# anilkeshwani/speech-integration

Hardware: AMD Instinct MI355X
Metric: train_tokens_per_sec (higher is better)
Workload: dtype bf16; 1 GPU; Llama-3.2-1B +5000 DSUs (V=133258), SFT step fwd+bwd+AdamW, seq_len=2048, batch=8/GPU, grad_accum=1, 16 layers, random-init weights, MLS-shaped synthetic DSU sequences; global_batch=8, seq_len=2048, parallelism=dp1

## Files before the change

speech-integration_amd/csrc/embed_ce.hip:

```cpp
#include "common_hip.h"

template <typename T>
__global__ __launch_bounds__(256) void embed_fwd_kernel(const int64_t* __restrict__ tokens, const T* __restrict__ table,
                                                        T* __restrict__ out, int64_t n_tok, int dim, int64_t vocab) {
    constexpr int N = Vec16<T>::N;
    const int nvec = dim / N;
    for (int64_t t = blockIdx.x; t < n_tok; t += gridDim.x) {
        const int64_t tok = tokens[t];
        const bool ok = tok >= 0 && tok < vocab;
        for (int v = threadIdx.x; v < nvec; v += 256) {
            Vec16<T> a;
            if (ok) a = load16(table + tok * dim + v * N);
            else
#pragma unroll
                for (int i = 0; i < N; ++i) a.set(i, 0.f);
            store16(out + t * dim + v * N, a);
        }
    }
}

extern "C" int ssi_embed_fwd(const int64_t* tokens, const void* table, void* out, int64_t n_tok, int64_t dim,
                             int64_t vocab, int dtype, void* stream) {
    if (n_tok == 0) return SSI_OK;
    SSI_CHECK_ARG(tokens && table && out && n_tok > 0 && dim > 0 && dim % 8 == 0 && vocab > 0);
    const unsigned grid = (unsigned)(n_tok < 65536 ? n_tok : 65536);
    SSI_DISPATCH_DTYPE(dtype, hipLaunchKernelGGL(embed_fwd_kernel<T>, dim3(grid), dim3(256), 0, (hipStream_t)stream, tokens,
                                                 (const T*)table, (T*)out, n_tok, (int)dim, vocab));
    SSI_LAUNCH_CHECK();
    return SSI_OK;
}

__global__ __launch_bounds__(256) void embed_index_kernel(const int64_t* __restrict__ tokens, int64_t n_tok, int64_t vocab,
                                                          int* __restrict__ first, int* __restrict__ count) {
    const int64_t t = (int64_t)blockIdx.x * 256 + threadIdx.x;
    if (t >= n_tok) return;
    const int64_t tok = tokens[t];
    if (tok < 0 || tok >= vocab) return;
    atomicMin(&first[tok], (int)t);
    atomicAdd(&count[tok], 1);
}

template <typename T, int MAXV>
__global__ __launch_bounds__(256) void embed_bwd_kernel(const int64_t* __restrict__ tokens, const T* __restrict__ dout,
                                                        T* __restrict__ dtable, int64_t n_tok, int dim, int64_t vocab,
                                                        const int* __restrict__ first, const int* __restrict__ count) {
    constexpr int N = Vec16<T>::N;
    const int lane = threadIdx.x & 63;
    const int64_t t0 = (int64_t)blockIdx.x * 4 + (threadIdx.x >> 6);
    if (t0 >= n_tok) return;
    const int64_t tok = tokens[t0];
    if (tok < 0 || tok >= vocab) return;
    if (first[tok] != (int)t0) return;
    const int need = count[tok];
    const int nvec = dim / N;
    float acc[MAXV][N];
#pragma unroll
    for (int k = 0; k < MAXV; ++k)
#pragma unroll
        for (int i = 0; i < N; ++i) acc[k][i] = 0.f;
    constexpr int SCAN = 8, ROWS = 8;
    __shared__ int hits_lds[4][64 * SCAN];
    int* hits = hits_lds[threadIdx.x >> 6];
    int found = 0;
    for (int64_t base0 = (t0 / 64) * 64; base0 < n_tok && found < need; base0 += 64 * SCAN) {
        int64_t tk[SCAN];
#pragma unroll
        for (int u = 0; u < SCAN; ++u) {
            const int64_t idx = base0 + 64 * u + lane;
            tk[u] = tokens[idx < n_tok ? idx : n_tok - 1];
        }
        int n = 0;
#pragma unroll
        for (int u = 0; u < SCAN; ++u) {
            const int64_t idx = base0 + 64 * u + lane;
            const bool hit = idx < n_tok && idx >= t0 && tk[u] == tok;
            const unsigned long long mask = __ballot(hit);
            if (hit) hits[n + __popcll(mask & ((1ull << lane) - 1ull))] = (int)(idx - base0);
            n += __popcll(mask);
        }
        __builtin_amdgcn_s_waitcnt(0xc07f);
        if (n == 1) {
            const T* src = dout + (base0 + hits[0]) * dim;
#pragma unroll
            for (int k = 0; k < MAXV; ++k) {
                const int v = lane + k * 64;
                const Vec16<T> r = load16(src + (v < nvec ? v : nvec - 1) * N);
#pragma unroll
                for (int i = 0; i < N; ++i) acc[k][i] += v < nvec ? r.get(i) : 0.f;
            }
        } else
        for (int h0 = 0; h0 < n; h0 += ROWS) {
            int pos[ROWS];
#pragma unroll
            for (int u = 0; u < ROWS; ++u) pos[u] = hits[h0 + u < n ? h0 + u : n - 1];
            Vec16<T> a[ROWS][MAXV];
#pragma unroll
            for (int u = 0; u < ROWS; ++u) {
                const T* src = dout + (base0 + pos[u]) * dim;
#pragma unroll
                for (int k = 0; k < MAXV; ++k) {
                    const int v = lane + k * 64;
                    a[u][k] = load16(src + (v < nvec ? v : nvec - 1) * N);
                }
            }
            __builtin_amdgcn_sched_barrier(0);
#pragma unroll
            for (int u = 0; u < ROWS; ++u) {
                const bool row_ok = h0 + u < n;
#pragma unroll
                for (int k = 0; k < MAXV; ++k) {
                    const bool ok = row_ok && lane + k * 64 < nvec;
#pragma unroll
                    for (int i = 0; i < N; ++i) acc[k][i] += ok ? a[u][k].get(i) : 0.f;
                }
            }
        }
        found += n;
    }
    T* dst = dtable + tok * dim;
#pragma unroll
    for (int k = 0; k < MAXV; ++k) {
        const int v = lane + k * 64;
        if (v < nvec) {
            Vec16<T> a = load16(dst + v * N);
#pragma unroll
            for (int i = 0; i < N; ++i) a.set(i, a.get(i) + acc[k][i]);
            store16(dst + v * N, a);
        }
    }
}

static inline int64_t embed_ws_vocab_slots(int64_t vocab) { return ssi_align_up(vocab, 64); }
extern "C" int64_t ssi_embed_bwd_workspace_bytes(int64_t vocab) { return 2 * embed_ws_vocab_slots(vocab) * (int64_t)sizeof(int); }

template <typename T>
static int launch_embed_bwd(const int64_t* tokens, const T* dout, T* dtable, int64_t n_tok, int dim, int64_t vocab,
                            const int* first, const int* count, hipStream_t st) {
    const int64_t vec_per_lane = ssi_cdiv(dim / Vec16<T>::N, 64);
    const dim3 grid((unsigned)ssi_cdiv(n_tok, 4));
    if (vec_per_lane <= 1) hipLaunchKernelGGL((embed_bwd_kernel<T, 1>), grid, dim3(256), 0, st, tokens, dout, dtable, n_tok, dim, vocab, first, count);
    else if (vec_per_lane <= 2) hipLaunchKernelGGL((embed_bwd_kernel<T, 2>), grid, dim3(256), 0, st, tokens, dout, dtable, n_tok, dim, vocab, first, count);
    else if (vec_per_lane <= 4) hipLaunchKernelGGL((embed_bwd_kernel<T, 4>), grid, dim3(256), 0, st, tokens, dout, dtable, n_tok, dim, vocab, first, count);
    else if (vec_per_lane <= 8) hipLaunchKernelGGL((embed_bwd_kernel<T, 8>), grid, dim3(256), 0, st, tokens, dout, dtable, n_tok, dim, vocab, first, count);
    else { ssi_set_error("embed_bwd: dim %d too large", dim); return SSI_ERR_UNSUPPORTED; }
    return SSI_OK;
}

extern "C" int ssi_embed_bwd(const int64_t* tokens, const void* dout, void* dtable, int64_t n_tok, int64_t dim,
                             int64_t vocab, int dtype, void* workspace, int64_t workspace_bytes, void* stream) {
    if (n_tok == 0) return SSI_OK;
    SSI_CHECK_ARG(tokens && dout && dtable && n_tok > 0 && n_tok < (1LL << 31) && dim > 0 && dim % 8 == 0 && vocab > 0);
    if (!workspace || workspace_bytes < ssi_embed_bwd_workspace_bytes(vocab)) { ssi_set_error("embed_bwd: workspace too small"); return SSI_ERR_WORKSPACE; }
    auto st = (hipStream_t)stream;
    int* first = (int*)workspace;
    int* count = first + embed_ws_vocab_slots(vocab);
    hipError_t e = hipMemsetAsync(first, 0x7f, embed_ws_vocab_slots(vocab) * sizeof(int), st);
    if (e == hipSuccess) e = hipMemsetAsync(count, 0, embed_ws_vocab_slots(vocab) * sizeof(int), st);
    if (e != hipSuccess) { ssi_set_error("embed_bwd: memset failed: %s", hipGetErrorString(e)); return SSI_ERR_HIP + (int)e; }
    hipLaunchKernelGGL(embed_index_kernel, dim3((unsigned)ssi_cdiv(n_tok, 256)), dim3(256), 0, st, tokens, n_tok, vocab, first, count);
    SSI_LAUNCH_CHECK();
    int rc = SSI_OK;
    SSI_DISPATCH_DTYPE(dtype, rc = launch_embed_bwd<T>(tokens, (const T*)dout, (T*)dtable, n_tok, (int)dim, vocab, first, count, st));
    if (rc) return rc;
    SSI_LAUNCH_CHECK();
    return SSI_OK;
}

enum CeMode { CE_PLAIN, CE_Z, CE_SMOOTH, CE_METRICS, CE_KL };

struct CeKl {
    const void* teacher = nullptr; int64_t ld_teacher = 0; const float* teacher_lse = nullptr; const float* row_kl_weight = nullptr;
    float beta = 0.f; float* row_kl = nullptr;
};

__device__ __forceinline__ bool ce_label_valid(int64_t label, int64_t vocab, int64_t ignore_index) {
    return label != ignore_index && label >= 0 && label < vocab;
}

template <typename T> __device__ __forceinline__ void ce_zero_row(T* lr, int64_t nvec) {
    constexpr int N = Vec16<T>::N;
    Vec16<T> z;
#pragma unroll
    for (int i = 0; i < N; ++i) z.set(i, 0.f);
    for (int64_t v = threadIdx.x; v < nvec; v += 512) store16(lr + v * N, z);
}

template <typename T> __device__ __forceinline__ float ce_row_lse(const T* lr, int64_t nvec, int64_t vocab, float* red) {
    constexpr int N = Vec16<T>::N;
    float m = -INFINITY, s = 0.f;
    for (int64_t v = threadIdx.x; v < nvec; v += 512) {
        Vec16<T> a = load16(lr + v * N);
        float lm = -INFINITY;
#pragma unroll
        for (int i = 0; i < N; ++i) if (v * N + i < vocab) lm = fmaxf(lm, a.get(i));
        if (lm > m) { s *= expf(m - lm); m = lm; }
#pragma unroll
        for (int i = 0; i < N; ++i) if (v * N + i < vocab) s += expf(a.get(i) - m);
    }
    const float gm = block_max(m, red);
    s = (m == -INFINITY) ? 0.f : s * expf(m - gm);
    const float gs = block_sum(s, red);
    return gm + logf(gs);
}

template <typename T> __device__ __forceinline__ float ce_row_sum(const T* lr, int64_t nvec, int64_t vocab, float* red) {
    constexpr int N = Vec16<T>::N;
    float s = 0.f;
    for (int64_t v = threadIdx.x; v < nvec; v += 512) {
        Vec16<T> a = load16(lr + v * N);
#pragma unroll
        for (int i = 0; i < N; ++i) if (v * N + i < vocab) s += a.get(i);
    }
    return block_sum(s, red);
}

template <typename T> __device__ __forceinline__ int ce_rank_row(const T* lr, int64_t nvec, int64_t vocab, int64_t label, float xl, int* redi) {
    constexpr int N = Vec16<T>::N;
    int cnt = 0;
    for (int64_t v = threadIdx.x; v < nvec; v += 512) {
        Vec16<T> a = load16(lr + v * N);
#pragma unroll
        for (int i = 0; i < N; ++i) {
            const int64_t c = v * N + i;
            const float x = a.get(i);
            cnt += (int)(c < vocab) & ((int)(x > xl) | ((int)(x == xl) & (int)(c < label)));
        }
    }
    return block_sum_i32(cnt, redi);
}

template <CeMode MODE, typename T>
__device__ __forceinline__ void ce_grad_row(T* lr, int64_t nvec, int64_t vocab, int64_t label, float lse, float w, float f, float ome, float wu) {
    constexpr int N = Vec16<T>::N;
    for (int64_t v = threadIdx.x; v < nvec; v += 512) {
        Vec16<T> a = load16(lr + v * N), o;
#pragma unroll
        for (int i = 0; i < N; ++i) {
            const int64_t c = v * N + i;
            float g = 0.f;
            if (c < vocab) {
                if constexpr (MODE == CE_PLAIN) g = w * (expf(a.get(i) - lse) - (c == label ? 1.f : 0.f));
                else g = w * (f * expf(a.get(i) - lse) - (c == label ? ome : 0.f));
                if constexpr (MODE == CE_SMOOTH) {
                    asm volatile("" : "+v"(g));
                    g -= wu;
                }
            }
            o.set(i, g);
        }
        store16(lr + v * N, o);
    }
}

template <typename T>
__device__ __forceinline__ void ce_kl_row(T* lr, const T* tr, int64_t nvec, int64_t nvec_t, int64_t vocab, int64_t label, float lse, float tlse,
                                          float w, float bk, int write_grad, double (&acc)[3]) {
    constexpr int N = Vec16<T>::N;
    acc[0] = acc[1] = acc[2] = 0.0;
    for (int64_t v = threadIdx.x; v < nvec; v += 512) {
        Vec16<T> a = load16(lr + v * N), o;
        Vec16<T> b = a;
        if (v < nvec_t) b = load16(tr + v * N);
#pragma unroll
        for (int i = 0; i < N; ++i) {
            const int64_t c = v * N + i;
            float g = 0.f;
            if (c < vocab) {
                const float x = a.get(i), t = b.get(i);
                const float p = expf(x - lse), q = expf(t - tlse);
                const double Q = exp((double)t - (double)tlse);
                acc[0] += Q * ((double)t - (double)x);
                acc[1] += Q;
                acc[2] += exp((double)x - (double)lse);
                g = w * (p - (c == label ? 1.f : 0.f)) + bk * (p - q);
            }
            o.set(i, g);
        }
        if (write_grad) store16(lr + v * N, o);
    }
}

template <typename T, CeMode MODE>
__device__ __forceinline__ void ce_generic_body(T* __restrict__ logits, int64_t ld, const int64_t* __restrict__ labels, int64_t vocab,
                                                int64_t ignore_index, float two_z, float ome, float e_over_v, float* __restrict__ row_loss,
                                                float* __restrict__ row_lse, float* __restrict__ row_z, float* __restrict__ row_u,
                                                float* __restrict__ row_nll, int32_t* __restrict__ row_rank, int write_grad,
                                                const float* __restrict__ row_weight, float* red, int* redi, const CeKl& kl = CeKl{}) {
    const int64_t row = blockIdx.x;
    T* lr = logits + row * ld;
    const int64_t label = labels[row];
    const int64_t nvec = ld / Vec16<T>::N;
    const bool valid = ce_label_valid(label, vocab, ignore_index);
    float lse = 0.f, sx = 0.f, w = 1.f, xl = 0.f;
    int cnt = -1;
    if (valid) {
        lse = ce_row_lse(lr, nvec, vocab, red);
        if constexpr (MODE == CE_SMOOTH) sx = ce_row_sum(lr, nvec, vocab, red);
        w = row_weight ? row_weight[row] : 1.f;
        if (MODE == CE_METRICS || threadIdx.x == 0) xl = to_f32<T>(lr[label]);
        if constexpr (MODE == CE_METRICS) cnt = ce_rank_row(lr, nvec, vocab, label, xl, redi);
    }
    if (threadIdx.x == 0) {
        row_loss[row] = w * (lse - xl);
        if (row_lse) row_lse[row] = lse;
        if constexpr (MODE == CE_Z) row_z[row] = w * (lse * lse);
        if constexpr (MODE == CE_SMOOTH) {
            if (row_z) row_z[row] = w * (lse * lse);
            row_u[row] = w * (lse - sx / (float)vocab);
        }
        if constexpr (MODE == CE_METRICS) { row_nll[row] = lse - xl; row_rank[row] = cnt; }
    }
    if constexpr (MODE == CE_KL) {
        if (!valid) {
            if (threadIdx.x == 0) kl.row_kl[row] = 0.f;
            if (write_grad) ce_zero_row(lr, nvec);
            return;
        }
        const float kw = kl.row_kl_weight ? kl.row_kl_weight[row] : w;
        __syncthreads();
        const float tlse = kl.teacher_lse[row];
        double acc[3];
        ce_kl_row<T>(lr, (const T*)kl.teacher + row * kl.ld_teacher, nvec, kl.ld_teacher / Vec16<T>::N, vocab, label, lse, tlse, w, kl.beta * kw,
                     write_grad, acc);
        __shared__ double redd[3][8];
#pragma unroll
        for (int q = 0; q < 3; ++q) acc[q] = wave_sum_f64(acc[q]);
        if ((threadIdx.x & 63) == 0) {
#pragma unroll
            for (int q = 0; q < 3; ++q) redd[q][threadIdx.x >> 6] = acc[q];
        }
        __syncthreads();
        if (threadIdx.x == 0) {
            double sum[3] = {0.0, 0.0, 0.0};
            for (int q = 0; q < 3; ++q)
                for (int i = 0; i < 8; ++i) sum[q] += redd[q][i];
            kl.row_kl[row] = kw * (float)(sum[0] / sum[1] - ((double)tlse - (double)lse) - log(sum[1]) + log(sum[2]));
        }
    } else if constexpr (MODE != CE_METRICS) {
        if (!write_grad) return;
        if (!valid) { ce_zero_row(lr, nvec); return; }
        const float f = fmaf(two_z, lse, 1.f);
        __syncthreads();
        ce_grad_row<MODE>(lr, nvec, vocab, label, lse, w, f, ome, w * e_over_v);
    }
}

template <typename T>
__global__ __launch_bounds__(512) void ce_fwd_kernel(T* __restrict__ logits, int64_t ld, const int64_t* __restrict__ labels,
                                                     int64_t vocab, int64_t ignore_index, float* __restrict__ row_loss,
                                                     float* __restrict__ row_lse, int write_grad, const float* __restrict__ row_weight) {
    __shared__ float red[16];
    ce_generic_body<T, CE_PLAIN>(logits, ld, labels, vocab, ignore_index, 0.f, 1.f, 0.f, row_loss, row_lse, nullptr, nullptr, nullptr, nullptr,
                                 write_grad, row_weight, red, nullptr);
}

template <typename T>
__global__ __launch_bounds__(512) void ce_fwd_z_kernel(T* __restrict__ logits, int64_t ld, const int64_t* __restrict__ labels,
                                                       int64_t vocab, int64_t ignore_index, float two_z, float* __restrict__ row_loss,
                                                       float* __restrict__ row_lse, float* __restrict__ row_z, int write_grad,
                                                       const float* __restrict__ row_weight) {
    __shared__ float red[16];
    ce_generic_body<T, CE_Z>(logits, ld, labels, vocab, ignore_index, two_z, 1.f, 0.f, row_loss, row_lse, row_z, nullptr, nullptr, nullptr,
                             write_grad, row_weight, red, nullptr);
}

template <typename T>
__global__ __launch_bounds__(512) void ce_fwd_smooth_kernel(T* __restrict__ logits, int64_t ld, const int64_t* __restrict__ labels,
                                                            int64_t vocab, int64_t ignore_index, float two_z, float ome, float e_over_v,
                                                            float* __restrict__ row_loss, float* __restrict__ row_lse,
                                                            float* __restrict__ row_z, float* __restrict__ row_u, int write_grad,
                                                            const float* __restrict__ row_weight) {
    __shared__ float red[16];
    ce_generic_body<T, CE_SMOOTH>(logits, ld, labels, vocab, ignore_index, two_z, ome, e_over_v, row_loss, row_lse, row_z, row_u, nullptr, nullptr,
                                  write_grad, row_weight, red, nullptr);
}

template <typename T>
__global__ __launch_bounds__(512) void ce_fwd_metrics_kernel(const T* __restrict__ logits, int64_t ld, const int64_t* __restrict__ labels,
                                                             int64_t vocab, int64_t ignore_index, float* __restrict__ row_loss,
                                                             float* __restrict__ row_lse, float* __restrict__ row_nll,
                                                             int32_t* __restrict__ row_rank, const float* __restrict__ row_weight) {
    __shared__ float red[16];
    __shared__ int redi[16];
    ce_generic_body<T, CE_METRICS>(const_cast<T*>(logits), ld, labels, vocab, ignore_index, 0.f, 1.f, 0.f, row_loss, row_lse, nullptr, nullptr,
                                   row_nll, row_rank, 0, row_weight, red, redi);
}

template <typename T>
__global__ __launch_bounds__(512) void ce_kl_generic_kernel(T* __restrict__ logits, int64_t ld, const int64_t* __restrict__ labels,
                                                            int64_t vocab, int64_t ignore_index, CeKl kl, float* __restrict__ row_loss,
                                                            float* __restrict__ row_lse, int write_grad,
                                                            const float* __restrict__ row_weight) {
    __shared__ float red[16];
    ce_generic_body<T, CE_KL>(logits, ld, labels, vocab, ignore_index, 0.f, 1.f, 0.f, row_loss, row_lse, nullptr, nullptr, nullptr, nullptr,
                              write_grad, row_weight, red, nullptr, kl);
}


template <int NCH, CeMode MODE, bool write_grad>
__device__ __forceinline__ void ce_row_bf16_body(bf16_t* __restrict__ logits, int64_t ld, const int64_t* __restrict__ labels, int64_t rows,
                                                 int64_t vocab, int64_t ignore_index, float two_z, float ome, float e_over_v,
                                                 float* __restrict__ row_loss, float* __restrict__ row_lse, float* __restrict__ row_z,
                                                 float* __restrict__ row_u, float* __restrict__ row_nll, int32_t* __restrict__ row_rank,
                                                 const float* __restrict__ row_weight, float* red, int* redi, const CeKl& kl = CeKl{}) {
    static_assert(MODE != CE_METRICS || !write_grad, "the metrics form writes no gradient");
    constexpr bool KL = MODE == CE_KL;
    constexpr int TD = NCH < 3 ? NCH : 3;
    constexpr bool WITH_F = MODE == CE_Z || MODE == CE_SMOOTH;
    constexpr bool SMOOTH = MODE == CE_SMOOTH;
    constexpr float LOG2E = 1.44269504088896340736f;
    constexpr int CHUNK = 8192;
    const int tid = threadIdx.x;
    const int voff = tid * 16;
    const int col0 = tid * 8;
    const int row_bytes = (int)(ld * 2);
    const int vocab_i = (int)vocab;
    u32x4 x[NCH];
    auto rsrc_of = [&](int64_t row) { return __builtin_amdgcn_make_buffer_rsrc(logits + row * ld, 0, row_bytes, 0x00020000u); };
    [[maybe_unused]] u32x4 tq[TD];
    auto lo = [](unsigned u) { return __builtin_bit_cast(float, u << 16); };
    auto hi = [](unsigned u) { return __builtin_bit_cast(float, u & 0xffff0000u); };
    auto opaque = [&]() {
#pragma unroll
        for (int c = 0; c < NCH; ++c)
#pragma unroll
            for (int d = 0; d < 4; ++d) asm volatile("" : "+v"(x[c][d]));
    };
    int64_t row = blockIdx.x;
    if (row >= rows) return;
    {
        const __amdgpu_buffer_rsrc_t r0 = rsrc_of(row);
#pragma unroll
        for (int c = 0; c < NCH; ++c) x[c] = __builtin_amdgcn_raw_buffer_load_b128(r0, voff, c * CHUNK * 2, 0);
    }
    for (; row < rows; row += gridDim.x) {
        const int64_t next = row + gridDim.x;
        const int64_t label = labels[row];
        const bool valid = ce_label_valid(label, vocab, ignore_index);
        const float w = row_weight ? row_weight[row] : 1.f;
        float log2w = row_weight ? __log2f(w) : 0.f;
        const __amdgpu_buffer_rsrc_t rs = rsrc_of(row);
        [[maybe_unused]] float kw = 0.f, bk = 0.f, dl = 0.f, nq = -INFINITY, klacc = 0.f;
        [[maybe_unused]] __amdgpu_buffer_rsrc_t rt = rs;
        if constexpr (KL) {
            kw = kl.row_kl_weight ? kl.row_kl_weight[row] : w;
            rt = __builtin_amdgcn_make_buffer_rsrc(const_cast<bf16_t*>((const bf16_t*)kl.teacher) + row * ld, 0, row_bytes, 0x00020000u);
        }
#pragma unroll
        for (int c = (NCH >= 2 ? NCH - 2 : 0); c < NCH; ++c) {
            const int left = vocab_i - c * CHUNK - col0;
#pragma unroll
            for (int d = 0; d < 4; ++d) {
                if (2 * d >= left) x[c][d] = (x[c][d] & 0xffff0000u) | 0x0000ff80u;
                if (2 * d + 1 >= left) x[c][d] = (x[c][d] & 0x0000ffffu) | 0xff800000u;
            }
        }
        float nl = -INFINITY;
        float wl = w;
        float wus = 0.f;
        unsigned flip = 0u;
        if (valid) {
            float xl = 0.f;
            if (MODE == CE_METRICS || tid == 0) xl = (float)logits[row * ld + label];
            float m = -INFINITY;
#pragma unroll
            for (int c = 0; c < NCH; ++c)
#pragma unroll
                for (int d = 0; d < 4; ++d) m = fmaxf(m, fmaxf(lo(x[c][d]), hi(x[c][d])));
            if constexpr (MODE != CE_METRICS) asm volatile("s_waitcnt vmcnt(0)" ::: "memory");
            const float gm = block_max(m, red);
            if constexpr (KL) {
#pragma unroll
                for (int i = 0; i < TD; ++i) tq[i] = __builtin_amdgcn_raw_buffer_load_b128(rt, voff, i * CHUNK * 2, 2 );
            }
            opaque();
            const float nm = -gm * LOG2E;
            float s = 0.f;
#pragma unroll
            for (int c = 0; c < NCH; ++c)
#pragma unroll
                for (int d = 0; d < 4; ++d)
                    s += __builtin_amdgcn_exp2f(fmaf(lo(x[c][d]), LOG2E, nm)) + __builtin_amdgcn_exp2f(fmaf(hi(x[c][d]), LOG2E, nm));
            const float gs = block_sum(s, red);
            const float lse = gm + logf(gs);
            float gsx = 0.f;
            if constexpr (SMOOTH) {
                opaque();
                float sx = 0.f;
#pragma unroll
                for (int c = 0; c < NCH; ++c) {
                    const int left = vocab_i - c * CHUNK - col0;
#pragma unroll
                    for (int d = 0; d < 4; ++d) {
                        if (c < NCH - 2) sx += lo(x[c][d]) + hi(x[c][d]);
                        else sx += (2 * d < left ? lo(x[c][d]) : 0.f) + (2 * d + 1 < left ? hi(x[c][d]) : 0.f);
                    }
                }
                gsx = block_sum(sx, red);
            }
            int cnt = 0;
            if constexpr (MODE == CE_METRICS) {
                opaque();
                const int below = (int)label - col0;
#pragma unroll
                for (int c = 0; c < NCH; ++c) {
                    const int b = below - c * CHUNK;
#pragma unroll
                    for (int d = 0; d < 4; ++d) {
                        const float a0 = lo(x[c][d]), a1 = hi(x[c][d]);
                        cnt += (int)(a0 > xl) | ((int)(a0 == xl) & (int)(2 * d < b));
                        cnt += (int)(a1 > xl) | ((int)(a1 == xl) & (int)(2 * d + 1 < b));
                    }
                }
                cnt = block_sum_i32(cnt, redi);
            }
            if (tid == 0) {
                row_loss[row] = w * (lse - xl);
                if (row_lse) row_lse[row] = lse;
                if constexpr (MODE == CE_Z) row_z[row] = w * (lse * lse);
                if constexpr (SMOOTH) {
                    if (row_z) row_z[row] = w * (lse * lse);
                    row_u[row] = w * (lse - gsx / (float)vocab_i);
                }
                if constexpr (MODE == CE_METRICS) { row_nll[row] = lse - xl; row_rank[row] = cnt; }
            }
            if constexpr (KL) {
                const float tlse = kl.teacher_lse[row];
                bk = kl.beta * kw;
                log2w = __log2f(w + bk);
                dl = tlse - lse;
                nq = -tlse * LOG2E;
            }
            nl = fmaf(-lse, LOG2E, log2w);
            if constexpr (WITH_F) {
                const float f = fmaf(two_z, lse, 1.f);
                nl += __log2f(fabsf(f));
                if constexpr (SMOOTH) { wl = w * ome; wus = w * e_over_v; }
                if (f < 0.f) { wl = -wl; wus = -wus; flip = 0x80008000u; }
            }
        } else {
            if constexpr (KL) {
#pragma unroll
                for (int i = 0; i < TD; ++i) tq[i] = u32x4{0u, 0u, 0u, 0u};
            }
            if (tid == 0) {
            row_loss[row] = 0.f;
            if (row_lse) row_lse[row] = 0.f;
            if constexpr (MODE == CE_Z) row_z[row] = 0.f;
            if constexpr (SMOOTH) { if (row_z) row_z[row] = 0.f; row_u[row] = 0.f; }
            if constexpr (MODE == CE_METRICS) { row_nll[row] = 0.f; row_rank[row] = -1; }
            }
        }
        opaque();
        const int hot = valid ? (int)label - col0 : -(1 << 30);
        const __amdgpu_buffer_rsrc_t rn = rsrc_of(next < rows ? next : row);
#pragma unroll
        for (int c = 0; c < NCH; ++c) {
            if constexpr (KL) {
                const u32x4 tc = tq[c % TD];
                const int left = vocab_i - c * CHUNK - col0;
                const int h = hot - c * CHUNK;
                float g[8];
#pragma unroll
                for (int e = 0; e < 8; ++e) {
                    const float xe = (e & 1) ? hi(x[c][e >> 1]) : lo(x[c][e >> 1]);
                    const float te = (e & 1) ? hi(tc[e >> 1]) : lo(tc[e >> 1]);
                    float q = __builtin_amdgcn_exp2f(fmaf(te, LOG2E, nq));
                    float term = q * ((te - xe) - dl);
                    if (c >= NCH - 2) {
                        q = e < left ? q : 0.f;
                        term = e < left ? term : 0.f;
                    }
                    klacc += term;
                    if (write_grad) {
                        const float pe = __builtin_amdgcn_exp2f(fmaf(xe, LOG2E, nl)) - (e == h ? wl : 0.f);
                        g[e] = pe - bk * q;
                    }
                }
                if (write_grad) {
                    bf16x8 ob;
#pragma unroll
                    for (int e = 0; e < 8; ++e) ob[e] = (bf16_t)g[e];
                    __builtin_amdgcn_raw_buffer_store_b128(__builtin_bit_cast(u32x4, ob), rs, voff, c * CHUNK * 2, 2 );
                }
                if (c + TD < NCH) tq[c % TD] = __builtin_amdgcn_raw_buffer_load_b128(rt, voff, (c + TD) * CHUNK * 2, 2 );
            } else if (write_grad) {
                float g[8];
#pragma unroll
                for (int d = 0; d < 4; ++d) {
                    g[2 * d] = __builtin_amdgcn_exp2f(fmaf(lo(x[c][d]), LOG2E, nl));
                    g[2 * d + 1] = __builtin_amdgcn_exp2f(fmaf(hi(x[c][d]), LOG2E, nl));
                }
                const int h = hot - c * CHUNK;
                if ((unsigned)h < 8u) {
#pragma unroll
                    for (int e = 0; e < 8; ++e) if (e == h) g[e] -= wl;
                }
                if constexpr (SMOOTH) {
                    const int left = vocab_i - c * CHUNK - col0;
#pragma unroll
                    for (int e = 0; e < 8; ++e) g[e] -= (c < NCH - 2 || e < left) ? wus : 0.f;
                }
                bf16x8 ob;
#pragma unroll
                for (int e = 0; e < 8; ++e) ob[e] = (bf16_t)g[e];
                u32x4 o = __builtin_bit_cast(u32x4, ob);
                if constexpr (WITH_F) {
#pragma unroll
                    for (int d = 0; d < 4; ++d) o[d] ^= flip;
                }
                __builtin_amdgcn_raw_buffer_store_b128(o, rs, voff, c * CHUNK * 2, 2 );
            }
            x[c] = __builtin_amdgcn_raw_buffer_load_b128(rn, voff, c * CHUNK * 2, 2 );
            __builtin_amdgcn_sched_barrier(0);
        }
        if constexpr (KL) {
            const float skl = block_sum(klacc, red);
            if (tid == 0) kl.row_kl[row] = valid ? kw * skl : 0.f;
        }
    }
}

template <int NCH, bool write_grad>
__global__ __launch_bounds__(1024, 4) void ce_row_bf16_kernel(bf16_t* __restrict__ logits, int64_t ld, const int64_t* __restrict__ labels,
                                                              int64_t rows, int64_t vocab, int64_t ignore_index,
                                                              float* __restrict__ row_loss, float* __restrict__ row_lse,
                                                              const float* __restrict__ row_weight) {
    __shared__ float red[16];
    ce_row_bf16_body<NCH, CE_PLAIN, write_grad>(logits, ld, labels, rows, vocab, ignore_index, 0.f, 1.f, 0.f, row_loss, row_lse, nullptr, nullptr,
                                                nullptr, nullptr, row_weight, red, nullptr);
}

template <int NCH, bool write_grad>
__global__ __launch_bounds__(1024, 4) void ce_row_bf16_z_kernel(bf16_t* __restrict__ logits, int64_t ld, const int64_t* __restrict__ labels,
                                                                int64_t rows, int64_t vocab, int64_t ignore_index, float two_z,
                                                                float* __restrict__ row_loss, float* __restrict__ row_lse,
                                                                float* __restrict__ row_z, const float* __restrict__ row_weight) {
    __shared__ float red[16];
    ce_row_bf16_body<NCH, CE_Z, write_grad>(logits, ld, labels, rows, vocab, ignore_index, two_z, 1.f, 0.f, row_loss, row_lse, row_z, nullptr,
                                            nullptr, nullptr, row_weight, red, nullptr);
}

template <int NCH, bool write_grad>
__global__ __launch_bounds__(1024, 4) void ce_row_bf16_smooth_kernel(bf16_t* __restrict__ logits, int64_t ld, const int64_t* __restrict__ labels,
                                                                     int64_t rows, int64_t vocab, int64_t ignore_index, float two_z, float ome,
                                                                     float e_over_v, float* __restrict__ row_loss, float* __restrict__ row_lse,
                                                                     float* __restrict__ row_z, float* __restrict__ row_u,
                                                                     const float* __restrict__ row_weight) {
    __shared__ float red[16];
    ce_row_bf16_body<NCH, CE_SMOOTH, write_grad>(logits, ld, labels, rows, vocab, ignore_index, two_z, ome, e_over_v, row_loss, row_lse, row_z,
                                                 row_u, nullptr, nullptr, row_weight, red, nullptr);
}

template <int NCH, bool write_grad>
__global__ __launch_bounds__(1024, 4) void ce_kl_row_bf16_kernel(bf16_t* __restrict__ logits, int64_t ld, const int64_t* __restrict__ labels,
                                                                 int64_t rows, int64_t vocab, int64_t ignore_index, CeKl kl,
                                                                 float* __restrict__ row_loss, float* __restrict__ row_lse,
                                                                 const float* __restrict__ row_weight) {
    __shared__ float red[16];
    ce_row_bf16_body<NCH, CE_KL, write_grad>(logits, ld, labels, rows, vocab, ignore_index, 0.f, 1.f, 0.f, row_loss, row_lse, nullptr, nullptr,
                                             nullptr, nullptr, row_weight, red, nullptr, kl);
}

template <int NCH>
__global__ __launch_bounds__(1024, 4) void ce_row_bf16_metrics_kernel(const bf16_t* __restrict__ logits, int64_t ld,
                                                                      const int64_t* __restrict__ labels, int64_t rows, int64_t vocab,
                                                                      int64_t ignore_index, float* __restrict__ row_loss,
                                                                      float* __restrict__ row_lse, float* __restrict__ row_nll,
                                                                      int32_t* __restrict__ row_rank, const float* __restrict__ row_weight) {
    __shared__ float red[16];
    __shared__ int redi[16];
    ce_row_bf16_body<NCH, CE_METRICS, false>(const_cast<bf16_t*>(logits), ld, labels, rows, vocab, ignore_index, 0.f, 1.f, 0.f, row_loss, row_lse,
                                             nullptr, nullptr, row_nll, row_rank, row_weight, red, redi);
}

static int ce_num_cus() {
    static const int n = [] {
        int dev = 0, cus = 0;
        if (hipGetDevice(&dev) != hipSuccess || hipDeviceGetAttribute(&cus, hipDeviceAttributeMultiprocessorCount, dev) != hipSuccess || cus <= 0) cus = 256;
        return cus;
    }();
    return n;
}

static bool ce_row_form(int dtype, const void* logits, int64_t ld, int64_t vocab) {
    const int64_t chunks = ssi_cdiv(ld, 8192);
    return dtype == SSI_BF16 && ((uintptr_t)logits & 15) == 0 && ld - vocab < 8192 && ld * 2 < (1LL << 31) &&
           (chunks <= 4 || chunks == 8 || (chunks >= 16 && chunks <= 18));
}
static dim3 ce_row_grid(int64_t rows) { return dim3((unsigned)(rows < ce_num_cus() ? rows : ce_num_cus())); }

#define SSI_CE_CHUNKS_CASE(n, ...) case n: { constexpr int N = n; __VA_ARGS__; } break;
#define SSI_CE_DISPATCH_CHUNKS(ld, ...)                                                                                                 \
    switch ((int)ssi_cdiv(ld, 8192)) {                                                                                                  \
        SSI_CE_CHUNKS_CASE(1, __VA_ARGS__) SSI_CE_CHUNKS_CASE(2, __VA_ARGS__) SSI_CE_CHUNKS_CASE(3, __VA_ARGS__)                        \
        SSI_CE_CHUNKS_CASE(4, __VA_ARGS__) SSI_CE_CHUNKS_CASE(8, __VA_ARGS__) SSI_CE_CHUNKS_CASE(16, __VA_ARGS__)                       \
        SSI_CE_CHUNKS_CASE(17, __VA_ARGS__) SSI_CE_CHUNKS_CASE(18, __VA_ARGS__)                                                         \
    }

struct CeArgs {
    void* logits; int64_t ld; const int64_t* labels; const float* row_weight; int64_t rows, vocab, ignore_index;
    float *row_loss, *row_lse; int write_grad, dtype; hipStream_t stream;
    float two_z = 0.f, ome = 1.f, e_over_v = 0.f;
    float *row_z = nullptr, *row_u = nullptr;
    float* row_nll = nullptr; int32_t* row_rank = nullptr;
    CeKl kl;
};

template <CeMode MODE, int NCH, bool write_grad> static void ce_launch_row(const CeArgs& a) {
    const dim3 grid = ce_row_grid(a.rows), block(1024);
    bf16_t* logits = (bf16_t*)a.logits;
    if constexpr (MODE == CE_PLAIN)
        hipLaunchKernelGGL((ce_row_bf16_kernel<NCH, write_grad>), grid, block, 0, a.stream, logits, a.ld, a.labels, a.rows, a.vocab, a.ignore_index,
                           a.row_loss, a.row_lse, a.row_weight);
    else if constexpr (MODE == CE_Z)
        hipLaunchKernelGGL((ce_row_bf16_z_kernel<NCH, write_grad>), grid, block, 0, a.stream, logits, a.ld, a.labels, a.rows, a.vocab, a.ignore_index,
                           a.two_z, a.row_loss, a.row_lse, a.row_z, a.row_weight);
    else if constexpr (MODE == CE_KL)
        hipLaunchKernelGGL((ce_kl_row_bf16_kernel<NCH, write_grad>), grid, block, 0, a.stream, logits, a.ld, a.labels, a.rows, a.vocab, a.ignore_index,
                           a.kl, a.row_loss, a.row_lse, a.row_weight);
    else if constexpr (MODE == CE_SMOOTH)
        hipLaunchKernelGGL((ce_row_bf16_smooth_kernel<NCH, write_grad>), grid, block, 0, a.stream, logits, a.ld, a.labels, a.rows, a.vocab,
                           a.ignore_index, a.two_z, a.ome, a.e_over_v, a.row_loss, a.row_lse, a.row_z, a.row_u, a.row_weight);
    else
        hipLaunchKernelGGL((ce_row_bf16_metrics_kernel<NCH>), grid, block, 0, a.stream, (const bf16_t*)logits, a.ld, a.labels, a.rows, a.vocab,
                           a.ignore_index, a.row_loss, a.row_lse, a.row_nll, a.row_rank, a.row_weight);
}

template <CeMode MODE, typename T> static void ce_launch_generic(const CeArgs& a) {
    const dim3 grid((unsigned)a.rows), block(512);
    T* logits = (T*)a.logits;
    if constexpr (MODE == CE_PLAIN)
        hipLaunchKernelGGL(ce_fwd_kernel<T>, grid, block, 0, a.stream, logits, a.ld, a.labels, a.vocab, a.ignore_index, a.row_loss, a.row_lse,
                           a.write_grad, a.row_weight);
    else if constexpr (MODE == CE_Z)
        hipLaunchKernelGGL(ce_fwd_z_kernel<T>, grid, block, 0, a.stream, logits, a.ld, a.labels, a.vocab, a.ignore_index, a.two_z, a.row_loss,
                           a.row_lse, a.row_z, a.write_grad, a.row_weight);
    else if constexpr (MODE == CE_KL)
        hipLaunchKernelGGL(ce_kl_generic_kernel<T>, grid, block, 0, a.stream, logits, a.ld, a.labels, a.vocab, a.ignore_index, a.kl, a.row_loss,
                           a.row_lse, a.write_grad, a.row_weight);
    else if constexpr (MODE == CE_SMOOTH)
        hipLaunchKernelGGL(ce_fwd_smooth_kernel<T>, grid, block, 0, a.stream, logits, a.ld, a.labels, a.vocab, a.ignore_index, a.two_z, a.ome,
                           a.e_over_v, a.row_loss, a.row_lse, a.row_z, a.row_u, a.write_grad, a.row_weight);
    else
        hipLaunchKernelGGL(ce_fwd_metrics_kernel<T>, grid, block, 0, a.stream, (const T*)logits, a.ld, a.labels, a.vocab, a.ignore_index, a.row_loss,
                           a.row_lse, a.row_nll, a.row_rank, a.row_weight);
}

template <CeMode MODE> static int ce_fwd_launch(const CeArgs& a) {
    SSI_CHECK_ARG(a.logits && a.labels && a.row_loss && a.rows >= 0 && a.vocab > 0 && a.ld >= a.vocab && a.ld % 8 == 0);
    SSI_CHECK_ARG(((uintptr_t)a.logits & 15) == 0);
    if constexpr (MODE == CE_KL) SSI_CHECK_ARG(((uintptr_t)a.kl.teacher & 15) == 0);
    if (a.rows == 0) return SSI_OK;
    bool row_form = ce_row_form(a.dtype, a.logits, a.ld, a.vocab);
    if constexpr (MODE == CE_KL) row_form = row_form && a.kl.ld_teacher == a.ld && ce_row_form(a.dtype, a.kl.teacher, a.kl.ld_teacher, a.vocab);
    if (row_form) {
        SSI_CE_DISPATCH_CHUNKS(a.ld,
            if (a.write_grad) ce_launch_row<MODE, N, true>(a);
            else ce_launch_row<MODE, N, false>(a));
    } else {
        SSI_DISPATCH_DTYPE(a.dtype, ce_launch_generic<MODE, T>(a));
    }
    SSI_LAUNCH_CHECK();
    return SSI_OK;
}

static bool ce_z_coeff_ok(float z) { return z >= 0.f && z <= 3.0e38f; }

extern "C" int ssi_ce_fwd_weighted(void* logits, int64_t ld, const int64_t* labels, const float* row_weight, int64_t rows, int64_t vocab,
                                   int64_t ignore_index, float* row_loss, float* row_lse, int write_grad, int dtype, void* stream) {
    return ce_fwd_launch<CE_PLAIN>(CeArgs{logits, ld, labels, row_weight, rows, vocab, ignore_index, row_loss, row_lse, write_grad, dtype, (hipStream_t)stream});
}

extern "C" int ssi_ce_fwd(void* logits, int64_t ld, const int64_t* labels, int64_t rows, int64_t vocab,
                          int64_t ignore_index, float* row_loss, float* row_lse, int write_grad, int dtype, void* stream) {
    return ssi_ce_fwd_weighted(logits, ld, labels, nullptr, rows, vocab, ignore_index, row_loss, row_lse, write_grad, dtype, stream);
}

extern "C" int ssi_ce_fwd_z(void* logits, int64_t ld, const int64_t* labels, const float* row_weight, int64_t rows, int64_t vocab,
                            int64_t ignore_index, float z_coeff, float* row_loss, float* row_lse, float* row_z, int write_grad, int dtype,
                            void* stream) {
    SSI_CHECK_ARG(row_z);
    if (!ce_z_coeff_ok(z_coeff)) {
        ssi_set_error("ce_fwd_z: z_coeff must be finite and >= 0, got %g", (double)z_coeff);
        return SSI_ERR_ARG;
    }
    CeArgs a{logits, ld, labels, row_weight, rows, vocab, ignore_index, row_loss, row_lse, write_grad, dtype, (hipStream_t)stream};
    a.two_z = 2.f * z_coeff;
    a.row_z = row_z;
    return ce_fwd_launch<CE_Z>(a);
}

extern "C" int ssi_ce_fwd_smooth(void* logits, int64_t ld, const int64_t* labels, const float* row_weight, int64_t rows, int64_t vocab,
                                 int64_t ignore_index, float smoothing, float z_coeff, float* row_loss, float* row_lse, float* row_u,
                                 float* row_z, int write_grad, int dtype, void* stream) {
    SSI_CHECK_ARG(row_u);
    if (!(smoothing >= 0.f) || !(smoothing < 1.f)) {
        ssi_set_error("ce_fwd_smooth: smoothing must be finite and in [0, 1), got %g", (double)smoothing);
        return SSI_ERR_ARG;
    }
    if (!ce_z_coeff_ok(z_coeff)) {
        ssi_set_error("ce_fwd_smooth: z_coeff must be finite and >= 0, got %g", (double)z_coeff);
        return SSI_ERR_ARG;
    }
    SSI_CHECK_ARG(row_z || z_coeff == 0.f);
    CeArgs a{logits, ld, labels, row_weight, rows, vocab, ignore_index, row_loss, row_lse, write_grad, dtype, (hipStream_t)stream};
    a.two_z = 2.f * z_coeff;
    a.ome = 1.f - smoothing, a.e_over_v = smoothing / (float)vocab;
    a.row_z = row_z, a.row_u = row_u;
    return ce_fwd_launch<CE_SMOOTH>(a);
}

extern "C" int ssi_ce_fwd_kl(void* logits, int64_t ld, const void* teacher, int64_t ld_teacher, const float* teacher_lse, const int64_t* labels,
                             const float* row_weight, const float* row_kl_weight, int64_t rows, int64_t vocab, int64_t ignore_index,
                             float kl_coeff, float* row_loss, float* row_lse, float* row_kl, int write_grad, int dtype, void* stream) {
    SSI_CHECK_ARG(teacher && teacher_lse && row_kl && teacher != logits && ld_teacher >= vocab && ld_teacher % 8 == 0);
    if (!ce_z_coeff_ok(kl_coeff)) {
        ssi_set_error("ce_fwd_kl: kl_coeff must be finite and >= 0, got %g", (double)kl_coeff);
        return SSI_ERR_ARG;
    }
    CeArgs a{logits, ld, labels, row_weight, rows, vocab, ignore_index, row_loss, row_lse, write_grad, dtype, (hipStream_t)stream};
    a.kl = CeKl{teacher, ld_teacher, teacher_lse, row_kl_weight, kl_coeff, row_kl};
    return ce_fwd_launch<CE_KL>(a);
}

extern "C" int ssi_ce_fwd_metrics(const void* logits, int64_t ld, const int64_t* labels, const float* row_weight, int64_t rows, int64_t vocab,
                                  int64_t ignore_index, float* row_loss, float* row_lse, float* row_nll, int32_t* row_rank, int dtype,
                                  void* stream) {
    SSI_CHECK_ARG(row_nll && row_rank);
    CeArgs a{const_cast<void*>(logits), ld, labels, row_weight, rows, vocab, ignore_index, row_loss, row_lse, 0, dtype, (hipStream_t)stream};
    a.row_nll = row_nll, a.row_rank = row_rank;
    return ce_fwd_launch<CE_METRICS>(a);
}

__global__ __launch_bounds__(1024) void ce_reduce_kernel(const float* __restrict__ row_loss, const int64_t* __restrict__ labels,
                                                         int64_t rows, int64_t vocab, int64_t ignore_index, float* __restrict__ out) {
    __shared__ float red[16];
    float s = 0.f, c = 0.f, bad = 0.f;
    for (int64_t r = threadIdx.x; r < rows; r += 1024) {
        const int64_t l = labels[r];
        if (ce_label_valid(l, vocab, ignore_index)) { s += row_loss[r]; c += 1.f; }
        else if (l != ignore_index) bad += 1.f;
    }
    s = block_sum(s, red);
    c = block_sum(c, red);
    bad = block_sum(bad, red);
    if (threadIdx.x == 0) { out[0] = s / c; out[1] = s; out[2] = c; out[3] = bad; }
}

extern "C" int ssi_ce_reduce(const float* row_loss, const int64_t* labels, int64_t rows, int64_t vocab, int64_t ignore_index,
                             float* out, void* stream) {
    SSI_CHECK_ARG(row_loss && labels && out && rows >= 0 && rows < (1LL << 24) && vocab > 0);
    hipLaunchKernelGGL(ce_reduce_kernel, dim3(1), dim3(1024), 0, (hipStream_t)stream, row_loss, labels, rows, vocab, ignore_index, out);
    SSI_LAUNCH_CHECK();
    return SSI_OK;
}

__device__ __forceinline__ void ce_metrics_add(double (&acc)[4], int rank, float nll, int topk) {
    acc[0] += 1.0;
    acc[1] += (double)nll;
    acc[2] += rank == 0 ? 1.0 : 0.0;
    acc[3] += rank < topk ? 1.0 : 0.0;
}

#define SSI_CE_MAX_RANGES 8
__global__ __launch_bounds__(1024) void ce_metrics_reduce_kernel(const float* __restrict__ row_nll, const int32_t* __restrict__ row_rank,
                                                                 const int64_t* __restrict__ labels, int64_t rows,
                                                                 const int64_t* __restrict__ ranges, int n_ranges, int topk, int accumulate,
                                                                 double* __restrict__ out) {
    __shared__ double red[4][16];
    const int wv = threadIdx.x >> 6, ln = threadIdx.x & 63;
    for (int j = 0; j <= n_ranges; ++j) {
        const bool all = j == n_ranges;
        const int64_t lo = all ? 0 : ranges[2 * j], hi = all ? 0 : ranges[2 * j + 1];
        double acc[4] = {0.0, 0.0, 0.0, 0.0};
        for (int64_t r = threadIdx.x; r < rows; r += 1024) {
            const int rank = row_rank[r];
            const int64_t l = labels[r];
            if (rank >= 0 && (all || (l >= lo && l <= hi))) ce_metrics_add(acc, rank, row_nll[r], topk);
        }
#pragma unroll
        for (int q = 0; q < 4; ++q) acc[q] = wave_sum_f64(acc[q]);
        __syncthreads();
        if (ln == 0) {
#pragma unroll
            for (int q = 0; q < 4; ++q) red[q][wv] = acc[q];
        }
        __syncthreads();
        if (threadIdx.x < 4) {
            double t = 0.0;
            for (int i = 0; i < 16; ++i) t += red[threadIdx.x][i];
            double* dst = out + 4 * j + threadIdx.x;
            *dst = accumulate ? *dst + t : t;
        }
    }
}

extern "C" int ssi_ce_metrics_reduce(const float* row_nll, const int32_t* row_rank, const int64_t* labels, int64_t rows, const int64_t* ranges,
                                     int n_ranges, int topk, int accumulate, double* out, void* stream) {
    SSI_CHECK_ARG(out && rows >= 0 && rows < (1LL << 31) && (rows == 0 || (row_nll && row_rank && labels)) && n_ranges >= 0 &&
                  n_ranges <= SSI_CE_MAX_RANGES && (ranges || n_ranges == 0) && topk >= 1);
    hipLaunchKernelGGL(ce_metrics_reduce_kernel, dim3(1), dim3(1024), 0, (hipStream_t)stream, row_nll, row_rank, labels, rows, ranges, n_ranges,
                       topk, accumulate, out);
    SSI_LAUNCH_CHECK();
    return SSI_OK;
}

__global__ __launch_bounds__(256) void seq_score_reduce_kernel(const float* __restrict__ row_nll, const int32_t* __restrict__ row_rank,
                                                               int64_t rows, const int64_t* __restrict__ seq_start,
                                                               const int64_t* __restrict__ seq_end, int64_t n_seq, int topk,
                                                               double* __restrict__ out) {
    const int ln = threadIdx.x & 63;
    const int64_t seq = (int64_t)blockIdx.x * 4 + (threadIdx.x >> 6);
    if (seq >= n_seq) return;
    int64_t end = seq_end[seq], start = seq_start[seq];
    end = end < 0 ? 0 : (end > rows ? rows : end);
    start = start < 0 ? 0 : (start > end ? end : start);
    double acc[4] = {0.0, 0.0, 0.0, 0.0};
    for (int64_t r = start + ln; r < end; r += 64) {
        const int rank = row_rank[r];
        if (rank >= 0) ce_metrics_add(acc, rank, row_nll[r], topk);
    }
#pragma unroll
    for (int q = 0; q < 4; ++q) acc[q] = wave_sum_f64(acc[q]);
    if (ln == 0) {
#pragma unroll
        for (int q = 0; q < 4; ++q) out[4 * seq + q] = acc[q];
    }
}

extern "C" int ssi_seq_score_reduce(const float* row_nll, const int32_t* row_rank, int64_t rows, const int64_t* seq_start,
                                    const int64_t* seq_end, int64_t n_seq, int topk, double* out, void* stream) {
    SSI_CHECK_ARG(rows >= 0 && rows < (1LL << 31) && n_seq >= 0 && n_seq < (1LL << 31) && topk >= 1 && (rows == 0 || (row_nll && row_rank)) &&
                  (n_seq == 0 || (seq_start && seq_end && out)));
    if (n_seq == 0) return SSI_OK;
    hipLaunchKernelGGL(seq_score_reduce_kernel, dim3((unsigned)ssi_cdiv(n_seq, 4)), dim3(256), 0, (hipStream_t)stream, row_nll, row_rank, rows,
                       seq_start, seq_end, n_seq, topk, out);
    SSI_LAUNCH_CHECK();
    return SSI_OK;
}
```

Measured before the change: 156,700 tokens/s.

## Give each unique token a full 256-thread block in embedding backward

The embedding backward kernel now assigns one 256-thread block per token position instead of one wave, so all four waves cooperate on scanning the token stream and on accumulating the gathered gradient rows. The index kernel stores n_tok - t with atomicMax so that both workspace arrays can be cleared with a single zero memset. A fast path handles tokens that occur only once, and the multi-hit path compacts hits across waves through shared memory with block barriers. This trades more blocks that exit immediately and extra syncthreads for wider parallelism on frequently repeated tokens. Embedding backward is a small part of a full training step.

```diff
diff --git a/speech-integration_amd/csrc/embed_ce.hip b/speech-integration_amd/csrc/embed_ce.hip
--- a/speech-integration_amd/csrc/embed_ce.hip
+++ b/speech-integration_amd/csrc/embed_ce.hip
@@ -36,91 +36,106 @@
     if (t >= n_tok) return;
     const int64_t tok = tokens[t];
     if (tok < 0 || tok >= vocab) return;
-    atomicMin(&first[tok], (int)t);
+    atomicMax(&first[tok], (int)(n_tok - t));
     atomicAdd(&count[tok], 1);
+}
+
+template <typename T, int KV, int R>
+__device__ __forceinline__ void embed_add_rows(const T* __restrict__ dout, int dim, int nvec, const int* hits, int h0, int n,
+                                               float (&acc)[KV][Vec16<T>::N]) {
+    constexpr int N = Vec16<T>::N;
+    Vec16<T> a[R][KV];
+#pragma unroll
+    for (int u = 0; u < R; ++u) {
+        const T* src = dout + (int64_t)hits[h0 + u < n ? h0 + u : n - 1] * dim;
+#pragma unroll
+        for (int k = 0; k < KV; ++k) {
+            const int v = (int)threadIdx.x + k * 256;
+            a[u][k] = load16(src + (v < nvec ? v : nvec - 1) * N);
+        }
+    }
+    __builtin_amdgcn_sched_barrier(0);
+#pragma unroll
+    for (int u = 0; u < R; ++u) {
+        const bool row_ok = h0 + u < n;
+#pragma unroll
+        for (int k = 0; k < KV; ++k) {
+            const bool ok = row_ok && (int)threadIdx.x + k * 256 < nvec;
+#pragma unroll
+            for (int i = 0; i < N; ++i) acc[k][i] += ok ? a[u][k].get(i) : 0.f;
+        }
+    }
 }
 
 template <typename T, int MAXV>
 __global__ __launch_bounds__(256) void embed_bwd_kernel(const int64_t* __restrict__ tokens, const T* __restrict__ dout,
                                                         T* __restrict__ dtable, int64_t n_tok, int dim, int64_t vocab,
                                                         const int* __restrict__ first, const int* __restrict__ count) {
-    constexpr int N = Vec16<T>::N;
-    const int lane = threadIdx.x & 63;
-    const int64_t t0 = (int64_t)blockIdx.x * 4 + (threadIdx.x >> 6);
-    if (t0 >= n_tok) return;
+    constexpr int N = Vec16<T>::N, KV = (MAXV + 3) / 4;
+    constexpr int SCAN = 16, ROWS = 32 / KV, TAIL = 4;
+    __shared__ int hits[256 * SCAN];
+    __shared__ int wave_hits[4];
+    const int lane = threadIdx.x & 63, wave = threadIdx.x >> 6;
+    const int64_t t0 = blockIdx.x;
     const int64_t tok = tokens[t0];
     if (tok < 0 || tok >= vocab) return;
-    if (first[tok] != (int)t0) return;
+    if (first[tok] != (int)(n_tok - t0)) return;
     const int need = count[tok];
     const int nvec = dim / N;
-    float acc[MAXV][N];
-#pragma unroll
-    for (int k = 0; k < MAXV; ++k)
+    float acc[KV][N];
+#pragma unroll
+    for (int k = 0; k < KV; ++k)
 #pragma unroll
         for (int i = 0; i < N; ++i) acc[k][i] = 0.f;
-    constexpr int SCAN = 8, ROWS = 8;
-    __shared__ int hits_lds[4][64 * SCAN];
-    int* hits = hits_lds[threadIdx.x >> 6];
-    int found = 0;
-    for (int64_t base0 = (t0 / 64) * 64; base0 < n_tok && found < need; base0 += 64 * SCAN) {
-        int64_t tk[SCAN];
-#pragma unroll
-        for (int u = 0; u < SCAN; ++u) {
-            const int64_t idx = base0 + 64 * u + lane;
-            tk[u] = tokens[idx < n_tok ? idx : n_tok - 1];
-        }
-        int n = 0;
-#pragma unroll
-        for (int u = 0; u < SCAN; ++u) {
-            const int64_t idx = base0 + 64 * u + lane;
-            const bool hit = idx < n_tok && idx >= t0 && tk[u] == tok;
-            const unsigned long long mask = __ballot(hit);
-            if (hit) hits[n + __popcll(mask & ((1ull << lane) - 1ull))] = (int)(idx - base0);
-            n += __popcll(mask);
-        }
-        __builtin_amdgcn_s_waitcnt(0xc07f);
-        if (n == 1) {
-            const T* src = dout + (base0 + hits[0]) * dim;
-#pragma unroll
-            for (int k = 0; k < MAXV; ++k) {
-                const int v = lane + k * 64;
-                const Vec16<T> r = load16(src + (v < nvec ? v : nvec - 1) * N);
-#pragma unroll
-                for (int i = 0; i < N; ++i) acc[k][i] += v < nvec ? r.get(i) : 0.f;
-            }
-        } else
-        for (int h0 = 0; h0 < n; h0 += ROWS) {
-            int pos[ROWS];
-#pragma unroll
-            for (int u = 0; u < ROWS; ++u) pos[u] = hits[h0 + u < n ? h0 + u : n - 1];
-            Vec16<T> a[ROWS][MAXV];
-#pragma unroll
-            for (int u = 0; u < ROWS; ++u) {
-                const T* src = dout + (base0 + pos[u]) * dim;
-#pragma unroll
-                for (int k = 0; k < MAXV; ++k) {
-                    const int v = lane + k * 64;
-                    a[u][k] = load16(src + (v < nvec ? v : nvec - 1) * N);
-                }
-            }
-            __builtin_amdgcn_sched_barrier(0);
-#pragma unroll
-            for (int u = 0; u < ROWS; ++u) {
-                const bool row_ok = h0 + u < n;
-#pragma unroll
-                for (int k = 0; k < MAXV; ++k) {
-                    const bool ok = row_ok && lane + k * 64 < nvec;
-#pragma unroll
-                    for (int i = 0; i < N; ++i) acc[k][i] += ok ? a[u][k].get(i) : 0.f;
-                }
-            }
-        }
-        found += n;
+    if (need == 1) {
+#pragma unroll
+        for (int k = 0; k < KV; ++k) {
+            const int v = (int)threadIdx.x + k * 256;
+            const Vec16<T> r = load16(dout + t0 * dim + (v < nvec ? v : nvec - 1) * N);
+#pragma unroll
+            for (int i = 0; i < N; ++i) acc[k][i] += v < nvec ? r.get(i) : 0.f;
+        }
+    } else {
+        int found = 0;
+        for (int64_t base = (t0 / 64) * 64; base < n_tok && found < need; base += 256 * SCAN) {
+            const int64_t wbase = base + (int64_t)wave * (64 * SCAN) + lane;
+            int64_t tk[SCAN];
+#pragma unroll
+            for (int u = 0; u < SCAN; ++u) {
+                const int64_t idx = wbase + 64 * u;
+                tk[u] = tokens[idx < n_tok ? idx : n_tok - 1];
+            }
+            int slot[SCAN], nw = 0;
+#pragma unroll
+            for (int u = 0; u < SCAN; ++u) {
+                const bool hit = wbase + 64 * u < n_tok && tk[u] == tok;
+                const unsigned long long mask = __ballot(hit);
+                slot[u] = hit ? nw + __popcll(mask & ((1ull << lane) - 1ull)) : -1;
+                nw += __popcll(mask);
+            }
+            if (lane == 0) wave_hits[wave] = nw;
+            __syncthreads();
+            int off = 0, n = 0;
+#pragma unroll
+            for (int w = 0; w < 4; ++w) {
+                const int c = wave_hits[w];
+                off += w < wave ? c : 0;
+                n += c;
+            }
+#pragma unroll
+            for (int u = 0; u < SCAN; ++u)
+                if (slot[u] >= 0) hits[off + slot[u]] = (int)(wbase + 64 * u);
+            __syncthreads();
+            int h0 = 0;
+            for (; h0 + TAIL < n; h0 += ROWS) embed_add_rows<T, KV, ROWS>(dout, dim, nvec, hits, h0, n, acc);
+            for (; h0 < n; h0 += TAIL) embed_add_rows<T, KV, TAIL>(dout, dim, nvec, hits, h0, n, acc);
+            found += n;
+        }
     }
     T* dst = dtable + tok * dim;
 #pragma unroll
-    for (int k = 0; k < MAXV; ++k) {
-        const int v = lane + k * 64;
+    for (int k = 0; k < KV; ++k) {
+        const int v = (int)threadIdx.x + k * 256;
         if (v < nvec) {
             Vec16<T> a = load16(dst + v * N);
 #pragma unroll
@@ -137,7 +152,7 @@
 static int launch_embed_bwd(const int64_t* tokens, const T* dout, T* dtable, int64_t n_tok, int dim, int64_t vocab,
                             const int* first, const int* count, hipStream_t st) {
     const int64_t vec_per_lane = ssi_cdiv(dim / Vec16<T>::N, 64);
-    const dim3 grid((unsigned)ssi_cdiv(n_tok, 4));
+    const dim3 grid((unsigned)n_tok);
     if (vec_per_lane <= 1) hipLaunchKernelGGL((embed_bwd_kernel<T, 1>), grid, dim3(256), 0, st, tokens, dout, dtable, n_tok, dim, vocab, first, count);
     else if (vec_per_lane <= 2) hipLaunchKernelGGL((embed_bwd_kernel<T, 2>), grid, dim3(256), 0, st, tokens, dout, dtable, n_tok, dim, vocab, first, count);
     else if (vec_per_lane <= 4) hipLaunchKernelGGL((embed_bwd_kernel<T, 4>), grid, dim3(256), 0, st, tokens, dout, dtable, n_tok, dim, vocab, first, count);
@@ -154,8 +169,7 @@
     auto st = (hipStream_t)stream;
     int* first = (int*)workspace;
     int* count = first + embed_ws_vocab_slots(vocab);
-    hipError_t e = hipMemsetAsync(first, 0x7f, embed_ws_vocab_slots(vocab) * sizeof(int), st);
-    if (e == hipSuccess) e = hipMemsetAsync(count, 0, embed_ws_vocab_slots(vocab) * sizeof(int), st);
+    const hipError_t e = hipMemsetAsync(first, 0, 2 * embed_ws_vocab_slots(vocab) * sizeof(int), st);
     if (e != hipSuccess) { ssi_set_error("embed_bwd: memset failed: %s", hipGetErrorString(e)); return SSI_ERR_HIP + (int)e; }
     hipLaunchKernelGGL(embed_index_kernel, dim3((unsigned)ssi_cdiv(n_tok, 256)), dim3(256), 0, st, tokens, n_tok, vocab, first, count);
     SSI_LAUNCH_CHECK();
```

Measured after the change: 156,800 tokens/s (median of 2 runs). About the same (+0.0%).
